# KochPJ/AutoPoseEstimation

Measured on AMD Instinct MI355X. Metric: RGB-D frames/sec (seg+DenseFusion+2-refine), 640x480 N=1000, higher is better.
Workload: dtype bf16x3

## Files before the change

autoposeestimation_amd/_lib.py:

```python
import ctypes
import os

import torch

_HERE = os.path.dirname(os.path.abspath(__file__))
LIB_PATH = os.environ.get("APE_HIP_LIB", os.path.join(_HERE, "libape_hip.so"))

_c = ctypes
_P, _I, _F, _L, _D = _c.c_void_p, _c.c_int, _c.c_float, _c.c_int64, _c.c_double

SIGNATURES = {
    "ape_abi_version": [],
    "ape_last_error": [],
    "ape_knn_f32": [_P, _P, _P, _I, _I, _I, _I, _I, _P],
    "ape_conv2d_nhwc_f32": [_P, _P, _P, _P, _P, _P, _P],
    "ape_packed_weights_bf16_elems": [_I, _I],
    "ape_pack_weights_bf16": [_P, _P, _I, _I, _P],
    "ape_conv2d_nhwc_bf16": [_P, _P, _P, _P, _P, _P, _I, _P],
    "ape_conv_gemm_supported": [_P],
    "ape_conv_gemm_bf16": [_P, _P, _P, _P, _P, _P, _I, _I, _P],
    "ape_pack_weights_s32k": [_P, _P, _I, _I, _P],
    "ape_convert_s32": [_P, _P, _c.c_long, _I, _I, _P],
    "ape_conv_gemm_s32_supported": [_P],
    "ape_conv_gemm_s32_debug": [_I],
    "ape_conv3x3_halo_s32_debug": [_I],
    "ape_conv_gemm_s32": [_P, _P, _P, _P, _I, _P, _I, _P, _P],
    "ape_conv_gemm_s32_per_image": [_P, _P, _c.c_long, _P, _P, _I, _P, _P],
    "ape_psp_fold_operands": [_P, _P, _P, _P, _P, _P, _P, _I, _I, _I, _I, _I, _I, _P],
    "ape_conv_gemm_bf16_fmt": [_P, _P, _P, _P, _P, _I, _P, _I, _I, _P],
    "ape_conv_gemm_splitk_workspace_bytes": [_P],
    "ape_conv_gemm_bf16_splitk": [_P, _P, _P, _P, _P, _P, _I, _P, _c.c_size_t, _P],
    "ape_conv_gemm_bf16_multi": [_I, _P, _P, _P, _P, _P, _I, _P],
    "ape_adaptive_avgpool_multi_nhwc_ld": [_P, _I, _P, _P, _I, _I, _I, _I, _I, _I, _P, _c.c_size_t, _P],
    "ape_upconv3x3_gather_ex": [_P, _P, _P, _I, _I, _I, _I, _I, _I, _F, _I, _P],
    "ape_upconv3x3_gather_strip_rows": [_I],
    "ape_upconv3x3_fused_supported": [_I, _I, _I, _I],
    "ape_upconv3x3_fused_debug": [_I],
    "ape_upconv3x3_fused_stamps": [_P],
    "ape_upconv3x3_fused_s32": [_P, _P, _P, _P, _I, _I, _I, _I, _I, _I, _F, _I, _P],
    "ape_upconv3x3_fused_seghead_s32": [_P, _P, _P, _I, _I, _I, _I, _I, _F, _I, _P, _P, _I, _P, _P, _I, _P],
    "ape_conv3x3_halo_s32_supported": [_P],
    "ape_conv3x3_halo_s32": [_P, _P, _P, _P, _I, _P, _I, _P, _P],
    "ape_conv3x3_halo_mx_supported": [_P],
    "ape_conv3x3_halo_mx": [_P, _P, _P, _P, _I, _P, _I, _P, _P],
    "ape_conv3x3_halo_mx_debug": [_I],
    "ape_s32_to_f16m6": [_P, _P, _c.c_long, _I, _P],
    "ape_stem_conv_pool_bf16": [_P, _P, _P, _P, _I, _I, _I, _I, _P],
    "ape_stem_conv_pool_u8": [_P, _I, _P, _P, _P, _P, _I, _I, _I, _I, _I, _I, _I, _P],
    "ape_conv3x3_halo_supported": [_P],
    "ape_conv3x3_halo_bf16": [_P, _P, _P, _P, _P, _P, _I, _P],
    "ape_maxpool3x3s2_nhwc_f32": [_P, _P, _I, _I, _I, _I, _P],
    "ape_adaptive_avgpool_nhwc_f32": [_P, _P, _I, _I, _I, _I, _I, _P],
    "ape_adaptive_avgpool_multi_workspace_bytes": [_I, _I],
    "ape_bilinear_nhwc_f32": [_P, _P, _I, _I, _I, _I, _I, _I, _I, _I, _I, _I, _I, _P],
    "ape_psp_prior_sum_f32": [_P, _P, _P, _P, _P, _I, _I, _I, _I, _P],
    "ape_upconv3x3_gather_f32": [_P, _P, _P, _I, _I, _I, _I, _I, _F, _P],
    "ape_gather_rows_f32": [_P, _P, _P, _I, _I, _I, _I, _P],
    "ape_ups_patch_gather_f32": [_P, _P, _P, _I, _I, _I, _I, _I, _P],
    "ape_log_softmax_rows_f32": [_P, _P, _c.c_long, _I, _P],
    "ape_mean_rows_f32": [_P, _P, _I, _I, _I, _P],
    "ape_pad3to4_f32": [_P, _P, _c.c_long, _P],
    "ape_head_select_f32": [_P, _I, _I, _I, _I, _P, _P, _P, _P, _P, _P, _P, _P, _I, _I, _I, _P],
    "ape_pose_select_f32": [_P, _P, _P, _P, _P, _I, _I, _P],
    "ape_head_conf_argmax_f32": [_P, _I, _I, _P, _P, _P, _P, _P, _P, _I, _P, _I, _I, _I, _P],
    "ape_pose_from_row_f32": [_P, _I, _I, _I, _P, _P, _P, _P, _P, _P, _P, _P, _P, _I, _I, _I, _P],
    "ape_pose_compose_f64": [_P, _P, _I, _P, _I, _I, _P],
    "ape_pose_recentre_f32": [_P, _P, _P, _I, _I, _P],
    "ape_adds_dis_f32": [_P, _P, _P, _P, _P, _I, _I, _I, _P, _P, _P, _P],
    "ape_adds_dis_batched_f32": [_P, _P, _P, _P, _I, _I, _I, _P, _P, _P],
    "ape_adds_select_f32": [_P, _P, _P, _P, _P, _P, _I, _F, _P, _P, _P],
    "ape_recentre_qt_f32": [_P, _P, _P, _I, _P],
    "ape_seg_argmax_f32": [_P, _I, _I, _P, _P, _c.c_long, _I, _P],
# ... 111 lines not shown


class ConvParams(_c.Structure):
    _fields_ = [(n, _c.c_int32) for n in ("B", "H", "W", "Cin", "ldx", "xoff", "Ho", "Wo", "Cout", "ldy", "yoff",
                                          "KH", "KW", "stride", "pad", "dil", "act")] + \
               [("alpha", _c.c_float), ("bias_bstride", _c.c_int32), ("ldr", _c.c_int32), ("roff", _c.c_int32), ("ups", _c.c_int32)]


class AugRotation(_c.Structure):
    _fields_ = [("a", _c.c_double * 6), ("fa", _c.c_int32 * 6), ("mode", _c.c_int32), ("reserved", _c.c_int32)]


class AugJitter(_c.Structure):
    _fields_ = [("n_ops", _c.c_int32), ("code", _c.c_int32 * 4), ("factor", _c.c_float * 4), ("shift", _c.c_int32 * 4)]


class BgsubTrainJob(_c.Structure):
    _fields_ = [("f_rgb", _c.c_void_p), ("b_rgb", _c.c_void_p), ("f_depth", _c.c_void_p), ("b_depth", _c.c_void_p), ("label", _c.c_void_p),
                ("rot", AugRotation), ("jit", AugJitter * 2), ("hflip", _c.c_int32), ("vflip", _c.c_int32)]


class SegTrainJob(_c.Structure):
    _fields_ = [("rgb", _c.c_void_p), ("label", _c.c_void_p), ("rot", AugRotation), ("jit", AugJitter), ("crop_x", _c.c_int32),
                ("crop_y", _c.c_int32), ("crop_side", _c.c_int32), ("class_id", _c.c_int32)]


class PoseTrainJob(_c.Structure):
    _fields_ = [("rgb", _c.c_void_p), ("depth", _c.c_void_p), ("label", _c.c_void_p), ("rot", AugRotation), ("add_t", _c.c_double * 3),
                ("out_off", _c.c_longlong), ("jit", AugJitter), ("rmin", _c.c_int32), ("rmax", _c.c_int32), ("cmin", _c.c_int32),
                ("cmax", _c.c_int32), ("ppx", _c.c_float), ("ppy", _c.c_float), ("fx", _c.c_float), ("fy", _c.c_float),
                ("depth_scale", _c.c_float), ("to_meter", _c.c_int32), ("add_noise", _c.c_int32)]


ACT_NONE, ACT_RELU, ACT_PRELU, ACT_SIGMOID = 0, 1, 2, 3
_RESTYPES = {"ape_last_error": _c.c_char_p, "ape_adaptive_avgpool_multi_workspace_bytes": _c.c_size_t, "ape_seg_components_workspace_bytes": _c.c_size_t,
             "ape_packed_weights_bf16_elems": _c.c_long, "ape_pc_batch_workspace_bytes": _c.c_size_t,
             "ape_conv2d_wgrad_workspace_bytes": _c.c_size_t, "ape_conv_gemm_splitk_workspace_bytes": _c.c_size_t,
             "ape_fpfh_workspace_bytes": _c.c_size_t, "ape_feature_nn1_workspace_bytes": _c.c_size_t, "ape_ransac_workspace_bytes": _c.c_size_t,
             "ape_fpfh_batch_workspace_bytes": _c.c_size_t, "ape_feature_nn1_batch_workspace_bytes": _c.c_size_t,
             "ape_ransac_batch_workspace_bytes": _c.c_size_t,
             "ape_bn_workspace_bytes": _c.c_size_t, "ape_jaccard_workspace_bytes": _c.c_size_t,
             "ape_bgsub_train_workspace_bytes": _c.c_size_t, "ape_seg_train_workspace_bytes": _c.c_size_t,
             "ape_seg_train_extents_offset": _c.c_size_t, "ape_seg_train_tables_offset": _c.c_size_t,
             "ape_pose_train_extents_offset": _c.c_size_t, "ape_pose_train_rows_offset": _c.c_size_t,
             "ape_pose_train_tables_offset": _c.c_size_t, "ape_pose_train_sel_offset": _c.c_size_t,
             "ape_pose_train_workspace_bytes": _c.c_size_t, "ape_pose_train_image_offset": _c.c_size_t,
             "ape_pose_train_sample_bytes": _c.c_size_t,
             "ape_linemod_box_workspace_bytes": _c.c_size_t, "ape_linemod_rows_offset": _c.c_size_t,
             "ape_linemod_tables_offset": _c.c_size_t, "ape_linemod_sel_offset": _c.c_size_t, "ape_linemod_workspace_bytes": _c.c_size_t}

_lib = None


ABI_VERSION = 11


class ApeError(RuntimeError):
    code = None


def lib():
    global _lib
    if _lib is None:
        if not os.path.exists(LIB_PATH):
            raise ImportError(
                "%s not found: build it with `python -c 'import __graft_entry__ as g; g.build()'` "
                "or `make -C autoposeestimation_amd/csrc` (hipcc, gfx950). There is no CPU fallback." % LIB_PATH)
        h = ctypes.CDLL(LIB_PATH)
        h.ape_abi_version.restype = _c.c_int
        if h.ape_abi_version() != ABI_VERSION:
            raise ImportError("%s is ABI %d, this package expects ABI %d: a stale library -- rebuild it with "
                              "`python -c 'import __graft_entry__ as g; g.build()'`" % (LIB_PATH, h.ape_abi_version(), ABI_VERSION))
        for name, argtypes in SIGNATURES.items():
            fn = getattr(h, name)
            fn.argtypes = argtypes
            fn.restype = _RESTYPES.get(name, _c.c_int)
        _lib = h
    return _lib


_raw_stream = getattr(torch._C, "_cuda_getCurrentRawStream", None)
_get_device = getattr(torch._C, "_cuda_getDevice", None) or torch.cuda.current_device


def stream_ptr():
    if _raw_stream is not None:
        return _c.c_void_p(_raw_stream(_get_device()))
    return _c.c_void_p(torch.cuda.current_stream().cuda_stream)


def dptr(t, dtype=None):
    if t is None:
        return _c.c_void_p(0)
    if not t.is_cuda:
        raise ApeError("tensor is on %s; the HIP path needs device memory (no CPU fallback)" % t.device)
    if not t.is_contiguous():
        raise ApeError("tensor must be contiguous")
    if dtype is not None and t.dtype != dtype:
        raise ApeError("expected %s, got %s" % (dtype, t.dtype))
    return _c.c_void_p(t.data_ptr())


def _failed(what, rc):
    msg = lib().ape_last_error()
    err = ApeError("%s failed: code %d (%s)" % (what, rc, msg.decode() if msg else ""))
    err.code = rc
    return err
# ... 28 lines not shown
```

autoposeestimation_amd/csrc/conv_gemm.hip:

```cpp
#include "common.h"
#include "s32.h"

namespace {

typedef __bf16 bf16x8 __attribute__((ext_vector_type(8)));
typedef float f32x4 __attribute__((ext_vector_type(4)));
typedef unsigned u32x4 __attribute__((ext_vector_type(4)));

struct GemmArgs {
    const float* x;
    const __bf16* w;
    const float* bias;
    const float* res;
    float* y;
    ape_conv_params p;
    int M, Kp, m_tiles, n_tiles, nk;
    int out_fmt;
    int dbg;
    long plane_stride;
    int nk_per;
    long split_stride;
};

__device__ __forceinline__ float activate(float v, int act, float alpha)
{
    if (act == APE_ACT_SIGMOID) return 1.f / (1.f + __expf(-v));
    const float neg = act == APE_ACT_RELU ? 0.f : (act == APE_ACT_PRELU ? alpha : 1.f) * v;
    return v > 0.f ? v : neg;
}

__device__ __forceinline__ void split8(const f32x4 v0, const f32x4 v1, bf16x8& hi, bf16x8& lo)
{
#pragma unroll
    for (int e = 0; e < 4; ++e) {
        hi[e] = (__bf16)v0[e];
        lo[e] = (__bf16)(v0[e] - (float)hi[e]);
        hi[4 + e] = (__bf16)v1[e];
        lo[4 + e] = (__bf16)(v1[e] - (float)hi[4 + e]);
    }
}

constexpr int BK = 32;

__device__ __forceinline__ int lds_off(int row, int c) { return row * BK + ((c ^ ((0 - (row >> 2)) & 3)) << 3); }

template <int NSPLIT, int BM, int BN, int WM, int WN, bool PURE, bool PP, bool SK>
__device__ __forceinline__ void conv_gemm_body(const GemmArgs& a, const int orig)
{
    static_assert(!PP || WM == 2, "the ping-pong schedule pairs the two row halves of an 8-wave block");
    constexpr int NT = WM * WN * 64;
    constexpr int NPL = NSPLIT == 3 ? 2 : 1;
    constexpr int WTM = BM / WM, WTN = BN / WN;
    constexpr int TM = WTM / 16, TN = WTN / 16;
    constexpr int A_IT = BM * 4 / NT;
    constexpr int B_IT = (BN * 4 + NT - 1) / NT;
    constexpr bool B_RAGGED = (BN * 4) % NT != 0;
    static_assert(BM * 4 % NT == 0 && A_IT >= 1 && B_IT >= 1, "staging shape");
    static_assert(WTM % 32 == 0 && WTN % 16 == 0 && BM % 64 == 0, "wave tile");

    constexpr size_t kStageElems = (size_t)NPL * (BM + BN) * BK;
    __shared__ __attribute__((aligned(16))) char smem_raw[2 * kStageElems * 2];
    __bf16* const S0 = reinterpret_cast<__bf16*>(smem_raw);
    auto a_tile = [&](int stage, int pl) { return S0 + stage * kStageElems + (size_t)pl * BM * BK; };
    auto b_tile = [&](int stage, int pl) { return S0 + stage * kStageElems + (size_t)NPL * BM * BK + (size_t)pl * BN * BK; };

    const ape_conv_params& p = a.p;
    const int nwg = a.m_tiles * a.n_tiles;
    const int xcd = orig % 8, q = nwg / 8, r = nwg % 8;
    const int logical = (xcd < r ? xcd * (q + 1) : r * (q + 1) + (xcd - r) * q) + orig / 8;
    const int n_tile = logical % a.n_tiles;
    const int m_tile = logical / a.n_tiles;
    const int m0 = m_tile * BM, n0 = n_tile * BN;

    const int tid = threadIdx.x;
    const int lane = tid & 63, wave = tid >> 6;
    const int wm = wave / WN, wn = wave % WN;
    const int HoWo = p.Ho * p.Wo;

    const int sc = tid & 3;
    const int srow = tid >> 2;
    unsigned a_off[A_IT];
    int a_iy0[PURE ? 1 : A_IT], a_ix0[PURE ? 1 : A_IT];
#pragma unroll
    for (int i = 0; i < A_IT; ++i) {
        int m = m0 + srow + i * (NT / 4);
        m = m < a.M ? m : a.M - 1;
        if (PURE) {
            a_off[i] = (unsigned)m * (unsigned)p.ldx + (unsigned)p.xoff + sc * 8;
        } else {
            const int b = m / HoWo, rem = m - b * HoWo;
            const int oy = rem / p.Wo, ox = rem - oy * p.Wo;
            a_iy0[i] = oy * p.stride - p.pad;
            a_ix0[i] = ox * p.stride - p.pad;
            a_off[i] = (unsigned)(b * p.H);
        }
// ... 33 lines not shown
                areg[i][1] = src[1];
            }
            kb = (unsigned)t_ci0;
            t_ci0 = t_ci0 + BK < p.Cin ? t_ci0 + BK : t_ci0;
        } else {
            const int dy = t_ky * p.dil, dx = t_kx * p.dil;
            a_ok = 0;
#pragma unroll
            for (int i = 0; i < A_IT; ++i) {
                const int iy = a_iy0[i] + dy, ix = a_ix0[i] + dx;
                const bool ok = (unsigned)iy < (unsigned)p.H && (unsigned)ix < (unsigned)p.W;
                const unsigned off = (unsigned)((((int)a_off[i] + clampi(iy, p.H - 1)) * p.W + clampi(ix, p.W - 1)) * p.ldx + p.xoff + t_ci0 + sc * 8);
                const f32x4* src = reinterpret_cast<const f32x4*>(a.x + off);
                areg[i][0] = src[0];
                areg[i][1] = src[1];
                a_ok |= ok ? (1u << i) : 0u;
            }
            kb = (unsigned)((t_ky * p.KW + t_kx) * p.Cin + t_ci0);
            if (++t_kx == p.KW) { t_kx = 0; if (++t_ky == p.KH) { t_ky = 0; t_ci0 = t_ci0 + BK < p.Cin ? t_ci0 + BK : t_ci0; } }
        }
#pragma unroll
        for (int pl = 0; pl < NPL; ++pl)
#pragma unroll
            for (int i = 0; i < B_IT; ++i)
                breg[pl][i] = *reinterpret_cast<const u32x4*>(a.w + pl * a.plane_stride + b_off[i] + kb);
    };
    auto store_tiles = [&](int stage) {
        const f32x4 z4 = {0.f, 0.f, 0.f, 0.f};
#pragma unroll
        for (int i = 0; i < A_IT; ++i) {
            const bool ok = PURE || ((a_ok >> i) & 1u);
            bf16x8 hi, lo;
            split8(ok ? areg[i][0] : z4, ok ? areg[i][1] : z4, hi, lo);
            const int o = lds_off(srow + i * (NT / 4), sc);
            *reinterpret_cast<bf16x8*>(a_tile(stage, 0) + o) = hi;
            if (NPL == 2) *reinterpret_cast<bf16x8*>(a_tile(stage, NPL - 1) + o) = lo;
        }
#pragma unroll
        for (int pl = 0; pl < NPL; ++pl)
#pragma unroll
            for (int i = 0; i < B_IT; ++i)
                if (!B_RAGGED || i + 1 < B_IT || srow + i * (NT / 4) < BN)
                    *reinterpret_cast<u32x4*>(b_tile(stage, pl) + lds_off(srow + i * (NT / 4), sc)) = breg[pl][i];
    };

    f32x4 acc[TM][TN];
#pragma unroll
    for (int i = 0; i < TM; ++i)
#pragma unroll
        for (int j = 0; j < TN; ++j)
#pragma unroll
            for (int e = 0; e < 4; ++e) acc[i][j][e] = 0.f;

    const int frow = lane & 15, fc = lane >> 4;
    const int a_row0 = wm * WTM + frow, b_row0 = wn * WTN + frow;
    bf16x8 bh[TN], bl[TN];
    auto read_b = [&](int stage) {
#pragma unroll
        for (int j = 0; j < TN; ++j) {
            const int o = lds_off(b_row0 + j * 16, fc);
            bh[j] = *reinterpret_cast<const bf16x8*>(b_tile(stage, 0) + o);
            if (NPL == 2) bl[j] = *reinterpret_cast<const bf16x8*>(b_tile(stage, NPL - 1) + o);
        }
    };
    constexpr int TMH = TM / 2;
    bf16x8 ah[TMH], al[TMH];
    auto read_a_rows = [&](int stage, int i0, int r0, int n) __attribute__((always_inline)) {
#pragma unroll
        for (int i = 0; i < n; ++i) {
            const int o = lds_off(a_row0 + (i0 + i) * 16, fc);
            ah[r0 + i] = *reinterpret_cast<const bf16x8*>(a_tile(stage, 0) + o);
            if (NPL == 2) al[r0 + i] = *reinterpret_cast<const bf16x8*>(a_tile(stage, NPL - 1) + o);
        }
    };
    auto read_a = [&](int stage, int i0) { read_a_rows(stage, i0, 0, TMH); };
    auto mfma_rows = [&](int i0, int r0, int n) __attribute__((always_inline)) {
#pragma unroll
        for (int i = r0; i < r0 + n; ++i)
#pragma unroll
            for (int j = 0; j < TN; ++j) {
                if (NPL == 2) {
                    acc[i0 + i][j] = __builtin_amdgcn_mfma_f32_16x16x32_bf16(bh[j], al[i], acc[i0 + i][j], 0, 0, 0);
                    acc[i0 + i][j] = __builtin_amdgcn_mfma_f32_16x16x32_bf16(bl[j], ah[i], acc[i0 + i][j], 0, 0, 0);
                }
                acc[i0 + i][j] = __builtin_amdgcn_mfma_f32_16x16x32_bf16(bh[j], ah[i], acc[i0 + i][j], 0, 0, 0);
            }
    };
    auto mfma_half = [&](int i0) {
#pragma unroll
        for (int i = 0; i < TMH; ++i)
#pragma unroll
            for (int j = 0; j < TN; ++j) {
                if (NPL == 2) {
                    acc[i0 + i][j] = __builtin_amdgcn_mfma_f32_16x16x32_bf16(bh[j], al[i], acc[i0 + i][j], 0, 0, 0);
                    acc[i0 + i][j] = __builtin_amdgcn_mfma_f32_16x16x32_bf16(bl[j], ah[i], acc[i0 + i][j], 0, 0, 0);
                }
                acc[i0 + i][j] = __builtin_amdgcn_mfma_f32_16x16x32_bf16(bh[j], ah[i], acc[i0 + i][j], 0, 0, 0);

            }
    };

    const int nk = SK ? (a.nk - kt0 < a.nk_per ? a.nk - kt0 : a.nk_per) : a.nk;
    if (NT == 512 && (a.dbg & 8) && __builtin_amdgcn_readfirstlane(threadIdx.x) >= 256) __builtin_amdgcn_s_setprio(1);
    load_tiles();
    store_tiles(0);
    load_tiles();
    __syncthreads();
    const bool behind = PP && __builtin_amdgcn_readfirstlane(wm) == 1;
    auto seg = [&]() {
        if (PP) {
            __builtin_amdgcn_sched_barrier(0);
            __syncthreads();
            __builtin_amdgcn_sched_barrier(0);
        }
    };
    if (behind) __syncthreads();
#pragma unroll 1
    for (int kt = 0; kt < nk; ++kt) {
        const int cur = kt & 1;
        read_b(cur);
        read_a(cur, 0);
        store_tiles(cur ^ 1);
        load_tiles();
        if constexpr (!PP && TMH % 2 == 0) {
            constexpr int Q = TMH / 2;
            mfma_rows(0, 0, Q);
            __builtin_amdgcn_sched_barrier(0);
            read_a_rows(cur, TMH, 0, Q);
            __builtin_amdgcn_sched_barrier(0);
            mfma_rows(0, Q, Q);
            __builtin_amdgcn_sched_barrier(0);
            read_a_rows(cur, TMH + Q, Q, Q);
            __builtin_amdgcn_sched_barrier(0);
            mfma_rows(TMH, 0, Q);
            mfma_rows(TMH, Q, Q);
        } else {
            seg();
            mfma_half(0);
            seg();
            read_a(cur, TMH);
            seg();
            mfma_half(TMH);
        }
        __syncthreads();
    }
    if (PP && !behind) __syncthreads();

    const bool vec_ok = (p.ldy % 4 == 0) && (p.yoff % 4 == 0) && (!a.res || (p.ldr % 4 == 0 && p.roff % 4 == 0));
    {
        const int nq = n0 + wn * WTN + fc * 4;
        const ape::ActFast af = ape::act_fast_make(p.act, p.alpha);
// ... 24 lines not shown
                const int n = nq + j * 16;
                if (!mok || n >= p.Cout) continue;
                float vv[4] = {acc[i][j][0], acc[i][j][1], acc[i][j][2], acc[i][j][3]};
                const int nvalid = min(4, p.Cout - n);
                if (vec_ok && nvalid == 4) {
                    if (brow) { vv[0] += brow[n]; vv[1] += brow[n + 1]; vv[2] += brow[n + 2]; vv[3] += brow[n + 3]; }
                    else if (a.bias) { vv[0] += b4[j].x; vv[1] += b4[j].y; vv[2] += b4[j].z; vv[3] += b4[j].w; }
                    if (a.res) { vv[0] += rr[j].x; vv[1] += rr[j].y; vv[2] += rr[j].z; vv[3] += rr[j].w; }
                    const float4 o4 = sigm ? make_float4(activate(vv[0], p.act, p.alpha), activate(vv[1], p.act, p.alpha), activate(vv[2], p.act, p.alpha),
                                                         activate(vv[3], p.act, p.alpha))
                                           : make_float4(ape::act_fast(vv[0], af), ape::act_fast(vv[1], af), ape::act_fast(vv[2], af), ape::act_fast(vv[3], af));
                    if (a.out_fmt == APE_FMT_S32) ape::s32_store4(yb, (long)m, p.ldy / 4, (p.yoff + n) / 4, o4);
                    else *reinterpret_cast<float4*>(yb + (size_t)m * p.ldy + p.yoff + n) = o4;
                } else {
                    for (int k = 0; k < nvalid; ++k) {
                        float t = vv[k];
                        if (a.bias) t += (brow ? brow : a.bias)[n + k];
                        if (a.res) t += a.res[(size_t)m * p.ldr + p.roff + n + k];
                        yb[(size_t)m * p.ldy + p.yoff + n + k] = activate(t, p.act, p.alpha);
                    }
                }
            }
        }
    }
}

template <int NSPLIT, int BM, int BN, int WM, int WN, bool PURE, bool PP>
__global__ __launch_bounds__(WM * WN * 64, 2) void conv_gemm_kernel(const GemmArgs a)
{
    conv_gemm_body<NSPLIT, BM, BN, WM, WN, PURE, PP, false>(a, (int)blockIdx.x);
}

template <int NSPLIT, bool PURE>
__global__ __launch_bounds__(256, 2) void conv_gemm_splitk_kernel(const GemmArgs a)
{
    conv_gemm_body<NSPLIT, 128, 128, 2, 2, PURE, false, true>(a, (int)blockIdx.x);
}

constexpr int kMultiMax = 4;
struct GemmMultiArgs {
    GemmArgs a[kMultiMax];
    int first[kMultiMax + 1];
};
template <int NSPLIT>
__global__ __launch_bounds__(256, 2) void conv_gemm_multi_kernel(const GemmMultiArgs m)
{
    const int blk = (int)blockIdx.x;
    int pi = 0;
#pragma unroll
    for (int i = 1; i < kMultiMax; ++i) pi = blk >= m.first[i] ? i : pi;
    conv_gemm_body<NSPLIT, 128, 128, 2, 2, true, false, false>(m.a[pi], blk - m.first[pi]);
}

template <int NSPLIT, int BM, int BN, int WM, int WN, bool PP = false>
void launch(GemmArgs& a, bool pure, hipStream_t st)
{
    a.m_tiles = ape::ceil_div(a.M, BM);
    a.n_tiles = ape::ceil_div(a.p.Cout, BN);
    if (pure)
        hipLaunchKernelGGL((conv_gemm_kernel<NSPLIT, BM, BN, WM, WN, true, PP>), dim3(a.m_tiles * a.n_tiles), dim3(WM * WN * 64), 0, st, a);
    else
        hipLaunchKernelGGL((conv_gemm_kernel<NSPLIT, BM, BN, WM, WN, false, PP>), dim3(a.m_tiles * a.n_tiles), dim3(WM * WN * 64), 0, st, a);
}

template <int NSPLIT>
void launch_splitk(GemmArgs& a, bool pure, hipStream_t st)
{
    a.m_tiles = ape::ceil_div(a.M, 128);
    a.n_tiles = ape::ceil_div(a.p.Cout, 128);
    const int gy = ape::ceil_div(a.nk, a.nk_per);
    if (pure)
        hipLaunchKernelGGL((conv_gemm_splitk_kernel<NSPLIT, true>), dim3(a.m_tiles * a.n_tiles, gy), dim3(256), 0, st, a);
    else
        hipLaunchKernelGGL((conv_gemm_splitk_kernel<NSPLIT, false>), dim3(a.m_tiles * a.n_tiles, gy), dim3(256), 0, st, a);
}

__global__ void splitk_finish_kernel(const float* __restrict__ ws, int splits, long M, int Cout, const float* __restrict__ bias, int bias_bstride,
                                     int HoWo, const float* __restrict__ res, int ldr, int roff, float* __restrict__ y, int ldy, int yoff, int act,
                                     float alpha)
{
    const long n = M * Cout;
    for (long i = blockIdx.x * (long)blockDim.x + threadIdx.x; i < n; i += (long)gridDim.x * blockDim.x) {
        const long m = i / Cout;
        const int c = (int)(i - m * Cout);
        float v = ws[i];
        for (int k = 1; k < splits; ++k) v += ws[(long)k * n + i];
        if (bias) v += bias[(bias_bstride ? (m / HoWo) * bias_bstride : 0) + c];
        if (res) v += res[m * ldr + roff + c];
        y[m * ldy + yoff + c] = activate(v, act, alpha);
    }
}

int splitk_tiles(const ape_conv_params& p, long M)
{
    const int nk = p.KH * p.KW * p.Cin / BK;
    const long tiles = (long)ape::ceil_div(M, 128) * ape::ceil_div(p.Cout, 128);
    if (p.Cout <= 64 || tiles >= 96 || nk < 8) return 0;
    long splits = ape::ceil_div(256L, tiles);
    splits = splits > nk / 4 ? nk / 4 : splits;
    splits = splits > 32 ? 32 : splits;
    if (splits < 2) return 0;
    return ape::ceil_div(nk, (int)splits);
}

bool supported(const ape_conv_params& p)
{
    if (p.B < 0 || p.H < 1 || p.W < 1 || p.Cin < 32 || p.Cin % 32 || p.Cout < 1 || p.KH < 1 || p.KW < 1 || p.stride < 1 ||
        p.dil < 1 || p.pad < 0 || p.Ho < 1 || p.Wo < 1 || p.ups != 0)
        return false;
    if (p.ldx % 4 || p.xoff % 4 || p.xoff + p.Cin > p.ldx || p.yoff + p.Cout > p.ldy) return false;
    if (p.act < APE_ACT_NONE || p.act > APE_ACT_SIGMOID) return false;
    const int ho = (p.H + 2 * p.pad - p.dil * (p.KH - 1) - 1) / p.stride + 1;
    const int wo = (p.W + 2 * p.pad - p.dil * (p.KW - 1) - 1) / p.stride + 1;
    if (ho != p.Ho || wo != p.Wo) return false;
    const long M = (long)p.B * p.Ho * p.Wo;
    if (M > (1L << 30) || (long)p.B * p.H * p.W * p.ldx >= (1L << 31) || (long)p.Cout * p.KH * p.KW * p.Cin >= (1L << 31)) return false;
    return true;
}

}

extern "C" int ape_conv_gemm_supported(const ape_conv_params* params) { return params && supported(*params) ? 1 : 0; }

extern "C" int ape_conv_gemm_bf16(const float* x, const void* w_packed, const float* bias, const float* residual, float* y,
                                  const ape_conv_params* params, int nsplit, int variant, void* stream)
{
    return ape_conv_gemm_bf16_fmt(x, w_packed, bias, residual, y, APE_FMT_F32, params, nsplit, variant, stream);
}

extern "C" int ape_conv_gemm_bf16_fmt(const float* x, const void* w_packed, const float* bias, const float* residual, void* y_, int out_fmt,
                                      const ape_conv_params* params, int nsplit, int variant, void* stream)
{
    float* y = (float*)y_;
    if (out_fmt != APE_FMT_F32 && out_fmt != APE_FMT_S32) return APE_EINVAL;
    if (out_fmt == APE_FMT_S32 && params && (params->ldy % 32 || params->Cout % 4 || params->yoff % 4 || (residual && (params->ldr % 4 || params->roff % 4))))
        return APE_EINVAL;
    if (!x || !w_packed || !y || !params || (nsplit != 1 && nsplit != 3) || variant < 0 || (variant & 15) > 6) return APE_EINVAL;
    const ape_conv_params& p = *params;
    if (!supported(p)) return APE_EINVAL;
    if (residual && p.roff + p.Cout > p.ldr) return APE_EINVAL;
    const long M = (long)p.B * p.Ho * p.Wo;
    if (M == 0) return APE_OK;
    GemmArgs a;
    a.x = x; a.w = (const __bf16*)w_packed; a.bias = bias; a.res = residual; a.y = y; a.p = p;
    a.M = (int)M;
    const int K = p.KH * p.KW * p.Cin;
    a.Kp = (K + 7) / 8 * 8;
    a.nk = K / BK;
    a.plane_stride = (long)p.Cout * a.Kp;
    a.dbg = variant >> 4;
    a.out_fmt = out_fmt;
    a.nk_per = 0;
    a.split_stride = 0;
    variant &= 15;
    const bool pure = p.KH == 1 && p.KW == 1 && p.stride == 1 && p.pad == 0;
    hipStream_t st = (hipStream_t)stream;
    if (variant == 0) {
        const int waste256 = ape::ceil_div(p.Cout, 256) * 256 - p.Cout;
        const int waste192 = ape::ceil_div(p.Cout, 192) * 192 - p.Cout;
        if (p.Cout <= 64) variant = 3;
        else if (p.Cout >= 256 && waste256 * 8 <= p.Cout && K >= 256 && (long)ape::ceil_div(M, 256) * ape::ceil_div(p.Cout, 256) >= 192) variant = 1;
        else if (p.Cout >= 192 && waste192 * 8 <= p.Cout && K >= 256 && (long)ape::ceil_div(M, 256) * ape::ceil_div(p.Cout, 192) >= 192) variant = 4;
        else variant = 2;
    }
    if (variant == 1) {
        if (nsplit == 3) launch<3, 256, 256, 2, 4>(a, pure, st); else launch<1, 256, 256, 2, 4>(a, pure, st);
    } else if (variant == 2) {
        if (nsplit == 3) launch<3, 128, 128, 2, 2>(a, pure, st); else launch<1, 128, 128, 2, 2>(a, pure, st);
    } else if (variant == 3) {
        if (nsplit == 3) launch<3, 256, 64, 4, 1>(a, pure, st); else launch<1, 256, 64, 4, 1>(a, pure, st);
    } else if (variant == 4) {
        if (nsplit == 3) launch<3, 256, 192, 2, 4>(a, pure, st); else launch<1, 256, 192, 2, 4>(a, pure, st);
    } else if (variant == 5) {
        if (nsplit == 3) launch<3, 256, 256, 2, 4, true>(a, pure, st); else launch<1, 256, 256, 2, 4, true>(a, pure, st);
    } else {
        if (nsplit == 3) launch<3, 128, 192, 2, 2>(a, pure, st); else launch<1, 128, 192, 2, 2>(a, pure, st);
    }
    return ape::check_launch("ape_conv_gemm_bf16");
}

extern "C" int ape_conv_gemm_bf16_multi(int n, const float* const* x, const void* const* w_packed, const float* const* bias, float* const* y,
                                        const ape_conv_params* params, int nsplit, void* stream)
{
    if (n < 1 || n > kMultiMax || !x || !w_packed || !y || !params || (nsplit != 1 && nsplit != 3)) return APE_EINVAL;
    GemmMultiArgs m;
    int total = 0;
    for (int i = 0; i < kMultiMax; ++i) {
        m.first[i] = total;
        if (i >= n) { m.a[i] = m.a[0]; continue; }
        const ape_conv_params& p = params[i];
        if (!x[i] || !w_packed[i] || !y[i] || !supported(p) || p.KH != 1 || p.KW != 1 || p.stride != 1 || p.pad != 0) return APE_EINVAL;
        const long M = (long)p.B * p.Ho * p.Wo;
        GemmArgs& a = m.a[i];
        a.x = x[i]; a.w = (const __bf16*)w_packed[i]; a.bias = bias ? bias[i] : nullptr; a.res = nullptr; a.y = y[i]; a.p = p;
        a.M = (int)M;
        a.Kp = (p.Cin + 7) / 8 * 8;
        a.nk = p.Cin / BK;
        a.plane_stride = (long)p.Cout * a.Kp;
        a.dbg = 0;
        a.out_fmt = APE_FMT_F32;
        a.nk_per = 0;
        a.split_stride = 0;
        a.m_tiles = ape::ceil_div(a.M, 128);
        a.n_tiles = ape::ceil_div(p.Cout, 128);
        total += a.m_tiles * a.n_tiles;
    }
    m.first[kMultiMax] = total;
    if (total == 0) return APE_OK;
    hipStream_t st = (hipStream_t)stream;
// ... 50 lines not shown
```

autoposeestimation_amd/csrc/runtime.hip:

```cpp
#include "common.h"
#include <string.h>

namespace ape {
static thread_local char g_err[256] = "";
void set_last_error(const char* what)
{
    strncpy(g_err, what ? what : "", sizeof(g_err) - 1);
    g_err[sizeof(g_err) - 1] = 0;
}
}

extern "C" int ape_abi_version(void) { return 11; }
extern "C" const char* ape_last_error(void) { return ape::g_err; }
```

autoposeestimation_amd/engine.py:

```python
import contextlib
import contextvars
import ctypes
import os

import torch

from . import _lib
from ._lib import ACT_NONE, ACT_PRELU, ACT_RELU, ACT_SIGMOID, ConvParams


def _st():
    return _lib.stream_ptr()


class LaunchProfile:

    def __init__(self, only=None):
        self.records = []
        self.only = only

    def wants(self, label):
        return self.only is None or label in self.only

    def begin(self, label):
# ... 163 lines not shown
        w, wp = pack_conv_weight(weight, device), None
        if nsplit:
            cout, kh, kw, cin = w.shape
            wp = torch.empty(_lib.lib().ape_packed_weights_bf16_elems(cout, kh * kw * cin), dtype=torch.bfloat16, device=device)
            _lib.call.ape_pack_weights_bf16(_lib.dptr(w), _lib.dptr(wp), cout, kh * kw * cin, _st())
        self._bind(w, wp, weight.shape[1], stride, pad, dil, act, alpha, precision, splitk)
        self.bias = None if bias is None else bias.detach().to(device=device, dtype=torch.float32).contiguous()

    @classmethod
    def from_packed(cls, w, wp, cin_real, stride=1, pad=0, dil=1, act=ACT_NONE, alpha=0.0, precision="f32", splitk=False):
        self = cls.__new__(cls)
        self._bind(w, wp, cin_real, stride, pad, dil, act, alpha, precision, splitk)
        self.bias = None
        return self

    def _bind(self, w, wp, cin_real, stride, pad, dil, act, alpha, precision, splitk):
        self.nsplit = _nsplit(precision)
        self.precision = precision
        self.w = w
        self.cout, self.kh, self.kw, self.cin = w.shape
        self.cin_real = cin_real
        if self.nsplit:
            if wp is None:
                raise ValueError("precision %s needs the packed bf16 planes" % precision)
            self.wp = wp
            self.variant = "conv_bf16_kernel<%d,%s>" % (self.nsplit, "128,128,2,2,64,false" if self.cout > 64 else "128,64,4,1,32,true")
        else:
            self.variant = "conv_f32_kernel<%s>" % ("128,2,2" if self.cout > 64 else "64,4,1" if self.cout > 32 else "32,4,1")
        self.stride, self.pad, self.dil, self.act, self.alpha = stride, pad, dil, act, float(alpha)
        self.splitk = bool(splitk)
        self._plans, self._ws32, self._wmx6 = {}, None, None

    def s32k(self):
        if self._ws32 is None:
            k = self.kh * self.kw * self.cin
            ws = torch.empty(self.cout * k * 2, dtype=torch.bfloat16, device=self.w.device)
            _lib.call.ape_pack_weights_s32k(_lib.dptr(self.w), _lib.dptr(ws), self.cout, k, _st())
            self._ws32 = ws
        return self._ws32

    def mx6k(self):
        if self._wmx6 is None:
            from . import mx6
            w = self.w.detach().float().cpu().numpy().reshape(self.cout, self.kh, self.kw, self.cin)
            lines = mx6.pack_lines(w.reshape(self.cout, self.kh * self.kw * (self.cin // 32), 32))
            self._wmx6 = torch.from_numpy(lines).to(self.w.device)
        return self._wmx6

    def _generic_variant(self, m):
        if self.nsplit and self.cout >= 256 and ((-(-self.cout // 256)) * 256 - self.cout) * 8 <= self.cout and m >= 65536:
            return "conv_bf16_kernel<%d,256,256,4,2,32,true>" % self.nsplit
        return self.variant

    def _gemm_variant(self, m):
        pure = "true" if (self.kh == 1 and self.kw == 1 and self.stride == 1 and self.pad == 0) else "false"
        v = GEMM_VARIANT & 15
        if v == 0:
            k = self.kh * self.kw * self.cin
            if self.cout <= 64:
                v = 3
            elif (self.cout >= 256 and ((-(-self.cout // 256)) * 256 - self.cout) * 8 <= self.cout and k >= 256
                  and -(-m // 256) * -(-self.cout // 256) >= 192):
                v = 1
            elif (self.cout >= 192 and ((-(-self.cout // 192)) * 192 - self.cout) * 8 <= self.cout and k >= 256
                  and -(-m // 256) * -(-self.cout // 192) >= 192):
                v = 4
            else:
                v = 2
        return "conv_gemm_kernel<%d,%s,%s,%s>" % (self.nsplit, {1: "256,256,2,4", 2: "128,128,2,2", 3: "256,64,4,1", 4: "256,192,2,4",
                                                               5: "256,256,2,4", 6: "128,192,2,2"}[v], pure, "true" if v == 5 else "false")

    def out_hw(self, h, w):
        ho = (h + 2 * self.pad - self.dil * (self.kh - 1) - 1) // self.stride + 1
        wo = (w + 2 * self.pad - self.dil * (self.kw - 1) - 1) // self.stride + 1
        return ho, wo

    def _make_plan(self, key):
        b, h, w, ldx, xoff, ldy, yoff, act, bias_bstride, ldr, roff, ups, splitk, in_fmt, out_fmt = key[:15]
        p = conv_params(self, b, h, w, ldx, ldy, xoff, yoff, act, bias_bstride, ldr, roff, ups)
        pref, L, m = ctypes.byref(p), _lib.lib(), b * p.Ho * p.Wo
        sk_bytes = 0
        if in_fmt == FMT_S32:
            if self.kh != 3:
                if not L.ape_conv_gemm_s32_supported(pref):
                    raise ValueError("no S32 kernel for this layer geometry (%dx%d, stride %d, Cin %d, Cout %d)" % (self.kh, self.kw, self.stride, self.cin, self.cout))
                args, entry, label = _ARGS_S32, "ape_conv_gemm_s32", gemm_s32_label(self.cout, ldr != 0)
            elif (USE_MX6 and self.cin in MX6_CIN and self.cout >= 128 and self.stride == 1 and xoff == 0 and ldx == self.cin
                  and L.ape_conv3x3_halo_mx_supported(pref)):
                args, entry, label = _ARGS_MX, "ape_conv3x3_halo_mx", halo_mx_label(self.dil)
            else:
                if not L.ape_conv3x3_halo_s32_supported(pref):
                    raise ValueError("no S32 kernel for this layer geometry (3x3, stride %d, dil %d, Cin %d, Cout %d)" % (self.stride, self.dil, self.cin, self.cout))
                args, entry, label = _ARGS_S32, "ape_conv3x3_halo_s32", halo_s32_label(self.dil)
        else:
            halo = bool(self.nsplit and USE_HALO_KERNEL and (ups or tiles16_mostly_full(h, w)) and L.ape_conv3x3_halo_supported(pref))
            gemm = bool(not halo and self.nsplit and USE_GEMM_KERNEL and L.ape_conv_gemm_supported(pref))
            if out_fmt == FMT_S32 and not gemm:
                raise ValueError("an S32 output from an fp32 input exists only on the conv_gemm kernel (Cin % 32 == 0, not a halo layer)")
            if halo:
                args, entry, label = _ARGS_BF16, "ape_conv3x3_halo_bf16", halo_label(self.nsplit, self.dil, self.cout, ups)
            elif gemm:
                sk_bytes = int(L.ape_conv_gemm_splitk_workspace_bytes(pref)) if splitk and out_fmt == FMT_F32 else 0
                args, entry = (_ARGS_SPLITK, "ape_conv_gemm_bf16_splitk") if sk_bytes else (_ARGS_GEMM, "ape_conv_gemm_bf16_fmt")
                label = self._gemm_variant(m)
            else:
                args, entry = (_ARGS_BF16, "ape_conv2d_nhwc_bf16") if self.nsplit else (_ARGS_F32, "ape_conv2d_nhwc_f32")
                label = self._generic_variant(m)
        hin, win = (h // 2, w // 2) if ups else (h, w)
        if len(self._plans) > 64:
            self._plans.clear()
        plan = self._plans[key] = (p, pref, args, getattr(_lib.call, entry), sk_bytes, label, conv_shape(self, b, p.Ho, p.Wo, ups),
                                   *_conv_cost(self, b, hin, win, p.Ho, p.Wo, ldr != 0))
        return plan

    def __call__(self, x, out=None, xoff=0, yoff=0, residual=None, roff=0, bias=None, bias_bstride=0, act=None, upsample2x=False,
                 out_fmt=FMT_F32, splitk=False):
        in_fmt = FMT_S32 if isinstance(x, S32) else FMT_F32
        if in_fmt == FMT_S32 or isinstance(residual, S32):
            if self.nsplit != 3:
                raise ValueError("S32 operands exist only in the split-bf16 ('bf16x3') precision")
            if in_fmt != FMT_S32:
                raise ValueError("S32 output / residual needs an S32 input on this path")
            if upsample2x:
                raise ValueError("no S32 kernel up-samples its input")
            x = x.t
        if upsample2x:
            can_fuse = (self.nsplit and USE_HALO_KERNEL and self.kh == 3 and self.kw == 3 and self.stride == 1 and self.pad == 1
                        and self.dil == 1 and self.cin % 32 == 0 and x.shape[3] == self.cin and xoff == 0)
            if not can_fuse:
                return self(bilinear(x, 2 * x.shape[1], 2 * x.shape[2], True), out, 0, yoff, residual, roff, bias, bias_bstride, act)
        b, h, w, ldx = x.shape
        if upsample2x:
            h, w = 2 * h, 2 * w
        ho, wo = self.out_hw(h, w)
        if out is None:
            out = torch.empty(b, ho, wo, self.cout, dtype=torch.float32, device=x.device)
        elif isinstance(out, S32):
            out = out.t
        if tuple(out.shape[:3]) != (b, ho, wo):
            raise ValueError("conv output buffer %s does not match %s" % (tuple(out.shape), (b, ho, wo)))
        res_fmt = FMT_F32
        if residual is not None:
            if isinstance(residual, S32):
                residual, res_fmt = residual.t, FMT_S32
            if tuple(residual.shape[:3]) != (b, ho, wo):
                raise ValueError("residual shape mismatch")
        bias = self.bias if bias is None else bias
        splitk = bool(splitk or (self.splitk and _POSE_STAGE.get()))
        key = (b, h, w, ldx, xoff, out.shape[3], yoff, self.act if act is None else act, bias_bstride, 0 if residual is None else residual.shape[3], roff,
               bool(upsample2x), splitk, in_fmt, out_fmt, USE_HALO_KERNEL, USE_GEMM_KERNEL, GEMM_VARIANT, USE_MX6, MX6_CIN)
        plan = self._plans.get(key) or self._make_plan(key)
        p, pref, args, fn, sk_bytes, label, shape, flop, nbytes = plan
        if p.alpha != self.alpha:
            p.alpha = self.alpha
        if args == _ARGS_MX:
            xq = torch.empty_like(x)
            _lib.call.ape_s32_to_f16m6(_lib.dptr(x, torch.float32), _lib.dptr(xq, torch.float32), b * h * w, ldx, _st())
# ... 581 lines not shown
```

include/ape_hip.h:

```cpp
#ifndef APE_HIP_H
#define APE_HIP_H

#include <stddef.h>
#include <stdint.h>

#ifdef __cplusplus
extern "C" {
#define APE_STATIC_ASSERT static_assert
#else
#define APE_STATIC_ASSERT _Static_assert
#endif

#define APE_OK 0
#define APE_EINVAL (-1)
#define APE_ELAUNCH (-2)
#define APE_EWORKSPACE (-3)

int ape_abi_version(void);
const char* ape_last_error(void);

int ape_knn_f32(const float* ref, const float* query, int64_t* idx,
                int batch, int dim, int ref_nb, int query_nb, int k, void* stream);

enum { APE_ACT_NONE = 0, APE_ACT_RELU = 1, APE_ACT_PRELU = 2, APE_ACT_SIGMOID = 3 };
typedef struct ape_conv_params {
    int32_t B, H, W, Cin, ldx, xoff;
    int32_t Ho, Wo, Cout, ldy, yoff;
    int32_t KH, KW, stride, pad, dil;
    int32_t act;
    float alpha;
    int32_t bias_bstride;
    int32_t ldr, roff;
    int32_t ups;
} ape_conv_params;
int ape_conv2d_nhwc_f32(const float* x, const float* w, const float* bias, const float* residual, float* y,
                        const ape_conv_params* params_host, void* stream);

long ape_packed_weights_bf16_elems(int cout, int K);
int ape_pack_weights_bf16(const float* w, void* out, int cout, int K, void* stream);
int ape_conv2d_nhwc_bf16(const float* x, const void* w_packed, const float* bias, const float* residual, float* y,
                         const ape_conv_params* params_host, int nsplit, void* stream);
int ape_conv_gemm_supported(const ape_conv_params* params_host);
int ape_conv_gemm_bf16(const float* x, const void* w_packed, const float* bias, const float* residual, float* y,
                       const ape_conv_params* params_host, int nsplit, int variant, void* stream);
enum { APE_FMT_F32 = 0, APE_FMT_S32 = 1 };
int ape_pack_weights_s32k(const float* w, void* out, int cout, int K, void* stream);
int ape_convert_s32(const void* x, void* y, long rows, int C, int to_s32, void* stream);
int ape_conv_gemm_s32_supported(const ape_conv_params* params_host);
int ape_conv3x3_halo_s32_debug(int bits);
int ape_conv_gemm_s32_debug(int bits);
int ape_conv_gemm_s32(const void* x_s32, const void* w_s32k, const float* bias, const void* residual, int res_fmt, void* y,
                      int out_fmt, const ape_conv_params* params_host, void* stream);
int ape_conv_gemm_s32_per_image(const void* x_s32, const void* w_s32k, long w_image_stride_bytes, const float* bias, void* y, int out_fmt,
                                const ape_conv_params* params_host, void* stream);
int ape_psp_fold_operands(const void* wf_s32k, const float* z1, const float* z2, const float* z3, const float* z6, void* w_out, void* x_s32,
                          int B, int h, int w, int ld, int Cin, int Cout, void* stream);
int ape_conv_gemm_bf16_fmt(const float* x, const void* w_packed, const float* bias, const float* residual, void* y, int out_fmt,
                           const ape_conv_params* params_host, int nsplit, int variant, void* stream);
int ape_conv_gemm_bf16_multi(int n, const float* const* x, const void* const* w_packed, const float* const* bias, float* const* y,
                             const ape_conv_params* params_host, int nsplit, void* stream);
size_t ape_conv_gemm_splitk_workspace_bytes(const ape_conv_params* params);
int ape_conv_gemm_bf16_splitk(const float* x, const void* w_packed, const float* bias, const float* residual, float* y,
                              const ape_conv_params* params, int nsplit, void* workspace, size_t workspace_bytes, void* stream);
int ape_adaptive_avgpool_multi_nhwc_ld(const void* x, int in_fmt, float* const* ys_host, const int* sizes_host, int nsizes, int B, int H, int W,
                                       int C, int ldx, void* workspace, size_t workspace_bytes, void* stream);
int ape_upconv3x3_gather_ex(const float* z, const float* bias, void* out, int out_fmt, int B, int h, int w, int C, int act, float alpha,
                            int fma, void* stream);
int ape_upconv3x3_gather_strip_rows(int rows);
int ape_upconv3x3_fused_supported(int h, int w, int Cin, int Cout);
int ape_upconv3x3_fused_stamps(void* device_buffer);
int ape_upconv3x3_fused_debug(int bits);
int ape_upconv3x3_fused_s32(const void* x_s32, const void* w9_s32k, const float* bias, void* out, int out_fmt, int B, int h, int w, int Cin,
                            int act, float alpha, int fma, void* stream);
int ape_upconv3x3_fused_seghead_s32(const void* x_s32, const void* w9_s32k, const float* bias, int B, int h, int w, int Cin, int act, float alpha,
                                    int fma, const float* head_w, const float* head_b, int C, uint8_t* label, float* score, int double_softmax,
                                    void* stream);
int ape_conv3x3_halo_s32_supported(const ape_conv_params* params_host);
int ape_conv3x3_halo_s32(const void* x_s32, const void* w_s32k, const float* bias, const void* residual, int res_fmt, void* y,
                         int out_fmt, const ape_conv_params* params_host, void* stream);
int ape_conv3x3_halo_mx_supported(const ape_conv_params* params_host);
int ape_conv3x3_halo_mx(const void* x_f16m6, const void* w_f16m6, const float* bias, const void* residual, int res_fmt, void* y,
                        int out_fmt, const ape_conv_params* params_host, void* stream);
int ape_conv3x3_halo_mx_debug(int bits);
int ape_s32_to_f16m6(const void* x_s32, void* y_f16m6, long pixels, int C, void* stream);
int ape_stem_conv_pool_bf16(const float* x, const float* w, const float* bias, float* y, int B, int H, int W, int nsplit,
                            void* stream);
int ape_stem_conv_pool_u8(const uint8_t* rgb, int n_frames, const int* rects, const float* w, const float* bias, float* y, int n, int Hf, int Wf,
                          int Hc, int Wc, int div255, int nsplit, void* stream);
int ape_conv3x3_halo_supported(const ape_conv_params* params_host);
int ape_conv3x3_halo_bf16(const float* x, const void* w_packed, const float* bias, const float* residual, float* y,
                          const ape_conv_params* params_host, int nsplit, void* stream);

int ape_maxpool3x3s2_nhwc_f32(const float* x, float* y, int B, int H, int W, int C, void* stream);
int ape_adaptive_avgpool_nhwc_f32(const float* x, float* y, int B, int H, int W, int C, int S, void* stream);
size_t ape_adaptive_avgpool_multi_workspace_bytes(int B, int C);
// ... 305 lines not shown
```

Baseline: 2145.

## Add single-wave 16x16 GEMM kernel for tiny-M pointwise convs

Adds a new conv_gemm_rows kernel that gives each 64-thread wave one 16x16 output tile, streaming K through an 8-deep register prefetch ring with split-bf16 MFMA. By default it is chosen for 1x1 convs with M<=64 rows and f32 output, such as the DenseFusion/refiner heads on N=1000 points after pooling. The aim is to replace large 128x128 block tiles, which leave most of the GPU idle and waste work on tiny M, with many small blocks. The MFMA helper is also moved into a shared header. The cost is less data reuse and a long serial K loop per wave.

```diff
diff --git a/autoposeestimation_amd/_lib.py b/autoposeestimation_amd/_lib.py
--- a/autoposeestimation_amd/_lib.py
+++ b/autoposeestimation_amd/_lib.py
@@ -18,6 +18,7 @@
     "ape_pack_weights_bf16": [_P, _P, _I, _I, _P],
     "ape_conv2d_nhwc_bf16": [_P, _P, _P, _P, _P, _P, _I, _P],
     "ape_conv_gemm_supported": [_P],
+    "ape_conv_gemm_rows_supported": [_P, _I, _I],
     "ape_conv_gemm_bf16": [_P, _P, _P, _P, _P, _P, _I, _I, _P],
     "ape_pack_weights_s32k": [_P, _P, _I, _I, _P],
     "ape_convert_s32": [_P, _P, _c.c_long, _I, _I, _P],
@@ -235,7 +236,7 @@
 _lib = None
 
 
-ABI_VERSION = 11
+ABI_VERSION = 12
 
 
 class ApeError(RuntimeError):
diff --git a/autoposeestimation_amd/csrc/conv_frag.h b/autoposeestimation_amd/csrc/conv_frag.h
--- /dev/null
+++ b/autoposeestimation_amd/csrc/conv_frag.h
@@ -0,0 +1,35 @@
+#pragma once
+#include <hip/hip_runtime.h>
+
+namespace ape {
+
+typedef __bf16 bf16x8 __attribute__((ext_vector_type(8)));
+typedef float f32x4 __attribute__((ext_vector_type(4)));
+
+constexpr int kFragK = 32;
+
+__device__ __forceinline__ void split8(const f32x4 v0, const f32x4 v1, bf16x8& hi, bf16x8& lo)
+{
+#pragma unroll
+    for (int e = 0; e < 4; ++e) {
+        hi[e] = (__bf16)v0[e];
+        lo[e] = (__bf16)(v0[e] - (float)hi[e]);
+        hi[4 + e] = (__bf16)v1[e];
+        lo[4 + e] = (__bf16)(v1[e] - (float)hi[4 + e]);
+    }
+}
+
+__device__ __forceinline__ int frag_row(int lane) { return lane & 15; }
+__device__ __forceinline__ int frag_chunk(int lane) { return lane >> 4; }
+
+template <bool SPLIT>
+__device__ __forceinline__ f32x4 mfma_tile(const bf16x8 w_hi, const bf16x8 w_lo, const bf16x8 a_hi, const bf16x8 a_lo, f32x4 acc)
+{
+    if (SPLIT) {
+        acc = __builtin_amdgcn_mfma_f32_16x16x32_bf16(w_hi, a_lo, acc, 0, 0, 0);
+        acc = __builtin_amdgcn_mfma_f32_16x16x32_bf16(w_lo, a_hi, acc, 0, 0, 0);
+    }
+    return __builtin_amdgcn_mfma_f32_16x16x32_bf16(w_hi, a_hi, acc, 0, 0, 0);
+}
+
+}
diff --git a/autoposeestimation_amd/csrc/conv_gemm.hip b/autoposeestimation_amd/csrc/conv_gemm.hip
--- a/autoposeestimation_amd/csrc/conv_gemm.hip
+++ b/autoposeestimation_amd/csrc/conv_gemm.hip
@@ -1,10 +1,12 @@
 #include "common.h"
+#include "conv_frag.h"
 #include "s32.h"
 
 namespace {
 
-typedef __bf16 bf16x8 __attribute__((ext_vector_type(8)));
-typedef float f32x4 __attribute__((ext_vector_type(4)));
+using ape::bf16x8;
+using ape::f32x4;
+using ape::split8;
 typedef unsigned u32x4 __attribute__((ext_vector_type(4)));
 
 struct GemmArgs {
@@ -29,18 +31,7 @@
     return v > 0.f ? v : neg;
 }
 
-__device__ __forceinline__ void split8(const f32x4 v0, const f32x4 v1, bf16x8& hi, bf16x8& lo)
-{
-#pragma unroll
-    for (int e = 0; e < 4; ++e) {
-        hi[e] = (__bf16)v0[e];
-        lo[e] = (__bf16)(v0[e] - (float)hi[e]);
-        hi[4 + e] = (__bf16)v1[e];
-        lo[4 + e] = (__bf16)(v1[e] - (float)hi[4 + e]);
-    }
-}
-
-constexpr int BK = 32;
+constexpr int BK = ape::kFragK;
 
 __device__ __forceinline__ int lds_off(int row, int c) { return row * BK + ((c ^ ((0 - (row >> 2)) & 3)) << 3); }
 
@@ -180,7 +171,7 @@
 #pragma unroll
             for (int e = 0; e < 4; ++e) acc[i][j][e] = 0.f;
 
-    const int frow = lane & 15, fc = lane >> 4;
+    const int frow = ape::frag_row(lane), fc = ape::frag_chunk(lane);
     const int a_row0 = wm * WTM + frow, b_row0 = wn * WTN + frow;
     bf16x8 bh[TN], bl[TN];
     auto read_b = [&](int stage) {
@@ -206,25 +197,14 @@
 #pragma unroll
         for (int i = r0; i < r0 + n; ++i)
 #pragma unroll
+            for (int j = 0; j < TN; ++j) acc[i0 + i][j] = ape::mfma_tile<NPL == 2>(bh[j], bl[j], ah[i], al[i], acc[i0 + i][j]);
+    };
+    auto mfma_half = [&](int i0) {
+#pragma unroll
+        for (int i = 0; i < TMH; ++i)
+#pragma unroll
             for (int j = 0; j < TN; ++j) {
-                if (NPL == 2) {
-                    acc[i0 + i][j] = __builtin_amdgcn_mfma_f32_16x16x32_bf16(bh[j], al[i], acc[i0 + i][j], 0, 0, 0);
-                    acc[i0 + i][j] = __builtin_amdgcn_mfma_f32_16x16x32_bf16(bl[j], ah[i], acc[i0 + i][j], 0, 0, 0);
-                }
-                acc[i0 + i][j] = __builtin_amdgcn_mfma_f32_16x16x32_bf16(bh[j], ah[i], acc[i0 + i][j], 0, 0, 0);
-            }
-    };
-    auto mfma_half = [&](int i0) {
-#pragma unroll
-        for (int i = 0; i < TMH; ++i)
-#pragma unroll
-            for (int j = 0; j < TN; ++j) {
-                if (NPL == 2) {
-                    acc[i0 + i][j] = __builtin_amdgcn_mfma_f32_16x16x32_bf16(bh[j], al[i], acc[i0 + i][j], 0, 0, 0);
-                    acc[i0 + i][j] = __builtin_amdgcn_mfma_f32_16x16x32_bf16(bl[j], ah[i], acc[i0 + i][j], 0, 0, 0);
-                }
-                acc[i0 + i][j] = __builtin_amdgcn_mfma_f32_16x16x32_bf16(bh[j], ah[i], acc[i0 + i][j], 0, 0, 0);
-
+                acc[i0 + i][j] = ape::mfma_tile<NPL == 2>(bh[j], bl[j], ah[i], al[i], acc[i0 + i][j]);
             }
     };
 
@@ -355,6 +335,97 @@
     conv_gemm_body<NSPLIT, 128, 128, 2, 2, true, false, false>(m.a[pi], blk - m.first[pi]);
 }
 
+constexpr int kRowsMax = 64;
+constexpr int kRowsDepth = 8;
+
+template <int NSPLIT>
+__global__ __launch_bounds__(64) void conv_gemm_rows_kernel(const GemmArgs a)
+{
+    constexpr int D = kRowsDepth;
+    constexpr bool SPLIT = NSPLIT == 3;
+    const ape_conv_params& p = a.p;
+    const int lane = threadIdx.x;
+    const int unit = (int)blockIdx.x;
+    const int mt = a.m_tiles;
+    const int n0 = (unit / mt) * 16, m0 = (unit % mt) * 16;
+    const int frow = ape::frag_row(lane), fc = ape::frag_chunk(lane);
+
+    int n = n0 + frow, m = m0 + frow;
+    n = n < p.Cout ? n : p.Cout - 1;
+    m = m < a.M ? m : a.M - 1;
+    const __bf16* const wp = a.w + (size_t)n * a.Kp + fc * 8;
+    const float* const xp = a.x + (size_t)m * p.ldx + p.xoff + fc * 8;
+    const int nk = a.nk;
+
+    bf16x8 wh[D], wl[D];
+    f32x4 x0[D], x1[D];
+    auto load = [&](int s, int t) {
+        t = t < nk ? t : nk - 1;
+        wh[s] = *reinterpret_cast<const bf16x8*>(wp + t * BK);
+        if (SPLIT) wl[s] = *reinterpret_cast<const bf16x8*>(wp + a.plane_stride + t * BK);
+        const f32x4* src = reinterpret_cast<const f32x4*>(xp + t * BK);
+        x0[s] = src[0];
+        x1[s] = src[1];
+    };
+    f32x4 acc = {0.f, 0.f, 0.f, 0.f};
+    auto use = [&](int s) {
+        bf16x8 ah, al;
+        split8(x0[s], x1[s], ah, al);
+        acc = ape::mfma_tile<SPLIT>(wh[s], wl[SPLIT ? s : 0], ah, al, acc);
+    };
+#pragma unroll
+    for (int s = 0; s < D; ++s) load(s, s);
+    int t0 = 0;
+#pragma unroll 1
+    for (; t0 + D <= nk; t0 += D) {
+#pragma unroll
+        for (int s = 0; s < D; ++s) {
+            use(s);
+            load(s, t0 + D + s);
+        }
+    }
+#pragma unroll
+    for (int s = 0; s < D; ++s)
+        if (t0 + s < nk) use(s);
+
+    const bool vec_ok = (p.ldy % 4 == 0) && (p.yoff % 4 == 0) && (!a.res || (p.ldr % 4 == 0 && p.roff % 4 == 0));
+    const int mo = m0 + frow, no = n0 + fc * 4;
+    if (mo >= a.M || no >= p.Cout) return;
+    const int HoWo = p.Ho * p.Wo;
+    const float* brow = (a.bias && p.bias_bstride) ? a.bias + (size_t)(mo / HoWo) * p.bias_bstride : nullptr;
+    float vv[4] = {acc[0], acc[1], acc[2], acc[3]};
+    const int nvalid = min(4, p.Cout - no);
+    if (vec_ok && nvalid == 4) {
+        const ape::ActFast af = ape::act_fast_make(p.act, p.alpha);
+        if (brow) { vv[0] += brow[no]; vv[1] += brow[no + 1]; vv[2] += brow[no + 2]; vv[3] += brow[no + 3]; }
+        else if (a.bias) { vv[0] += a.bias[no]; vv[1] += a.bias[no + 1]; vv[2] += a.bias[no + 2]; vv[3] += a.bias[no + 3]; }
+        if (a.res) {
+            const float4 rr = *reinterpret_cast<const float4*>(a.res + (size_t)mo * p.ldr + p.roff + no);
+            vv[0] += rr.x; vv[1] += rr.y; vv[2] += rr.z; vv[3] += rr.w;
+        }
+        const float4 o4 = p.act == APE_ACT_SIGMOID
+                              ? make_float4(activate(vv[0], p.act, p.alpha), activate(vv[1], p.act, p.alpha), activate(vv[2], p.act, p.alpha),
+                                            activate(vv[3], p.act, p.alpha))
+                              : make_float4(ape::act_fast(vv[0], af), ape::act_fast(vv[1], af), ape::act_fast(vv[2], af), ape::act_fast(vv[3], af));
+        *reinterpret_cast<float4*>(a.y + (size_t)mo * p.ldy + p.yoff + no) = o4;
+    } else {
+        for (int k = 0; k < nvalid; ++k) {
+            float t = vv[k];
+            if (a.bias) t += (brow ? brow : a.bias)[no + k];
+            if (a.res) t += a.res[(size_t)mo * p.ldr + p.roff + no + k];
+            a.y[(size_t)mo * p.ldy + p.yoff + no + k] = activate(t, p.act, p.alpha);
+        }
+    }
+}
+
+template <int NSPLIT>
+void launch_rows(GemmArgs& a, hipStream_t st)
+{
+    a.m_tiles = ape::ceil_div(a.M, 16);
+    a.n_tiles = ape::ceil_div(a.p.Cout, 16);
+    hipLaunchKernelGGL((conv_gemm_rows_kernel<NSPLIT>), dim3(a.m_tiles * a.n_tiles), dim3(64), 0, st, a);
+}
+
 template <int NSPLIT, int BM, int BN, int WM, int WN, bool PP = false>
 void launch(GemmArgs& a, bool pure, hipStream_t st)
 {
@@ -421,9 +492,23 @@
     return true;
 }
 
+bool rows_take(const ape_conv_params& p, int out_fmt)
+{
+    const bool pure = p.KH == 1 && p.KW == 1 && p.stride == 1 && p.pad == 0;
+    const long M = (long)p.B * p.Ho * p.Wo;
+    return supported(p) && pure && M >= 1 && M <= kRowsMax && out_fmt == APE_FMT_F32;
+}
+
 }
 
 extern "C" int ape_conv_gemm_supported(const ape_conv_params* params) { return params && supported(*params) ? 1 : 0; }
+
+extern "C" int ape_conv_gemm_rows_supported(const ape_conv_params* params, int out_fmt, int has_residual)
+{
+    if (!params || !rows_take(*params, out_fmt)) return 0;
+    if (has_residual && params->roff + params->Cout > params->ldr) return 0;
+    return 1;
+}
 
 extern "C" int ape_conv_gemm_bf16(const float* x, const void* w_packed, const float* bias, const float* residual, float* y,
                                   const ape_conv_params* params, int nsplit, int variant, void* stream)
@@ -438,7 +523,7 @@
     if (out_fmt != APE_FMT_F32 && out_fmt != APE_FMT_S32) return APE_EINVAL;
     if (out_fmt == APE_FMT_S32 && params && (params->ldy % 32 || params->Cout % 4 || params->yoff % 4 || (residual && (params->ldr % 4 || params->roff % 4))))
         return APE_EINVAL;
-    if (!x || !w_packed || !y || !params || (nsplit != 1 && nsplit != 3) || variant < 0 || (variant & 15) > 6) return APE_EINVAL;
+    if (!x || !w_packed || !y || !params || (nsplit != 1 && nsplit != 3) || variant < 0 || (variant & 15) > 7) return APE_EINVAL;
     const ape_conv_params& p = *params;
     if (!supported(p)) return APE_EINVAL;
     if (residual && p.roff + p.Cout > p.ldr) return APE_EINVAL;
@@ -458,6 +543,12 @@
     variant &= 15;
     const bool pure = p.KH == 1 && p.KW == 1 && p.stride == 1 && p.pad == 0;
     hipStream_t st = (hipStream_t)stream;
+    if (variant == 7 && !rows_take(p, out_fmt)) return APE_EINVAL;
+    if (variant == 0 && rows_take(p, out_fmt)) variant = 7;
+    if (variant == 7) {
+        if (nsplit == 3) launch_rows<3>(a, st); else launch_rows<1>(a, st);
+        return ape::check_launch("ape_conv_gemm_bf16");
+    }
     if (variant == 0) {
         const int waste256 = ape::ceil_div(p.Cout, 256) * 256 - p.Cout;
         const int waste192 = ape::ceil_div(p.Cout, 192) * 192 - p.Cout;
diff --git a/autoposeestimation_amd/csrc/runtime.hip b/autoposeestimation_amd/csrc/runtime.hip
--- a/autoposeestimation_amd/csrc/runtime.hip
+++ b/autoposeestimation_amd/csrc/runtime.hip
@@ -10,5 +10,5 @@
 }
 }
 
-extern "C" int ape_abi_version(void) { return 11; }
+extern "C" int ape_abi_version(void) { return 12; }
 extern "C" const char* ape_last_error(void) { return ape::g_err; }
diff --git a/autoposeestimation_amd/engine.py b/autoposeestimation_amd/engine.py
--- a/autoposeestimation_amd/engine.py
+++ b/autoposeestimation_amd/engine.py
@@ -239,9 +239,11 @@
             return "conv_bf16_kernel<%d,256,256,4,2,32,true>" % self.nsplit
         return self.variant
 
-    def _gemm_variant(self, m):
+    def _gemm_variant(self, m, pref=None, out_fmt=FMT_F32, residual=False):
         pure = "true" if (self.kh == 1 and self.kw == 1 and self.stride == 1 and self.pad == 0) else "false"
         v = GEMM_VARIANT & 15
+        if v == 7 or (v == 0 and pref is not None and _lib.lib().ape_conv_gemm_rows_supported(pref, out_fmt, int(bool(residual)))):
+            return "conv_gemm_rows_kernel<%d>" % self.nsplit
         if v == 0:
             k = self.kh * self.kw * self.cin
             if self.cout <= 64:
@@ -289,7 +291,7 @@
             elif gemm:
                 sk_bytes = int(L.ape_conv_gemm_splitk_workspace_bytes(pref)) if splitk and out_fmt == FMT_F32 else 0
                 args, entry = (_ARGS_SPLITK, "ape_conv_gemm_bf16_splitk") if sk_bytes else (_ARGS_GEMM, "ape_conv_gemm_bf16_fmt")
-                label = self._gemm_variant(m)
+                label = self._gemm_variant(m) if sk_bytes else self._gemm_variant(m, pref, out_fmt, ldr != 0)
             else:
                 args, entry = (_ARGS_BF16, "ape_conv2d_nhwc_bf16") if self.nsplit else (_ARGS_F32, "ape_conv2d_nhwc_f32")
                 label = self._generic_variant(m)
diff --git a/include/ape_hip.h b/include/ape_hip.h
--- a/include/ape_hip.h
+++ b/include/ape_hip.h
@@ -41,6 +41,7 @@
 int ape_conv2d_nhwc_bf16(const float* x, const void* w_packed, const float* bias, const float* residual, float* y,
                          const ape_conv_params* params_host, int nsplit, void* stream);
 int ape_conv_gemm_supported(const ape_conv_params* params_host);
+int ape_conv_gemm_rows_supported(const ape_conv_params* params_host, int out_fmt, int has_residual);
 int ape_conv_gemm_bf16(const float* x, const void* w_packed, const float* bias, const float* residual, float* y,
                        const ape_conv_params* params_host, int nsplit, int variant, void* stream);
 enum { APE_FMT_F32 = 0, APE_FMT_S32 = 1 };
```

After: 2152 (median of 6 runs). No clear change (+0.3%).
